# cosdata/cosdata

Hardware: AMD Instinct MI355X
Metric: QPS at recall@10≥0.95, 1024-dim dense cosine, 1/2/4/8 MI355X (higher is better)
Workload: dtype u8

## Files before the change

### cosdata_amd/csrc/engine.hip

```cpp
#include <hip/hip_runtime.h>

#include <algorithm>
#include <cstdarg>
#include <cstdio>
#include <cstdlib>
#include <chrono>
#include <cmath>
#include <condition_variable>
#include <cstring>
#include <map>
#include <mutex>
#include <string>
#include <thread>
#include <vector>

#include "engine_internal.h"

using namespace cosdev;

static thread_local std::string g_err;
int32_t cos_fail(int32_t code, const char *fmt, ...) {
    char buf[512];
    va_list ap;
    va_start(ap, fmt);
    vsnprintf(buf, sizeof(buf), fmt, ap);
    va_end(ap);
    g_err = buf;
    return code;
}

extern "C" const char *cos_last_error_string(void) { return g_err.c_str(); }

extern "C" int32_t cos_device_count(int32_t *out) {
    if (!out) return cos_fail(COS_ERR_INVALID, "null argument");
    int n = 0;
    hipError_t e = hipGetDeviceCount(&n);
    if (e != hipSuccess) { *out = 0; return cos_fail(COS_ERR_NO_DEVICE, "hipGetDeviceCount: %s", hipGetErrorString(e)); }
    *out = n;
    return COS_OK;
}

static u32 pow2ceil(u32 v) { u32 p = 1; while (p < v) p <<= 1; return p; }

int32_t cos_set_device(const cos_index *ix) {
    HIP_TRY(hipSetDevice(ix->p.device));
    return COS_OK;
}

static bool graph_ready(const cos_index *ix) {
// ... 600 lines not shown
                const u32 *row = &adj[(size_t)v * M];
                for (u32 j = M; j-- > 0;) {
                    const u32 u = row[j];
                    if (u != cosdev::ROW_EMPTY && u < n && !seen[u]) stack.push_back(u);
                }
            }
        };
        dfs_from(n - 1);
        for (u32 v = 0; v < n; v++) if (!seen[v]) dfs_from(v);
        HIP_TRY(ix->d_order_rank[kl].alloc(n));
        HIP_TRY(hipMemcpy(ix->d_order_rank[kl], rank.data(), (size_t)n * 4, hipMemcpyHostToDevice));
        ix->order_rank_n[kl] = n;
    }
    ix->order_rank_valid = true;
    return COS_OK;
}

static void clear_current_table(cos_index *ix) {
    ix->d_tcodes = nullptr;
    ix->d_tmags = nullptr;
    ix->d_tcsums = nullptr;
    ix->table_cols = 0;
    ix->table_level_min = 0;
    ix->table_stride = 0;
}
static u32 walk_table_max_cols(const cos_index *ix) {
    const long long env = cosdev::tune_or(cosdev::TUNE_WALK_TABLE_COLS, -1);
    return env >= 0 ? (u32)std::min<long long>(env, 1ll << 20) : ix->walk_table_max_cols;
}
static u32 walk_table_min_B(const cos_index *ix) {
    const long long env = cosdev::tune_or(cosdev::TUNE_WALK_TABLE_MIN_B, -1);
    return env >= 0 ? (u32)std::min<long long>(env, 0xFFFFFFFFll) : ix->walk_table_min_B;
}
static constexpr long long WALK_TABLE_EARLY_WGS_DEFAULT = 0;
static constexpr long long WALK_UP_TABLE_DEFAULT = 1;
cosdev::WalkPlanIn cos_walk_plan_in(const cos_index *ix, u32 B, u32 ef) {
    cosdev::WalkPlanIn in{};
    in.eng = ix->eng;
    in.storage = ix->p.storage;
    in.nchunks = ix->nchunks;
    in.G = ix->G;
    in.num_layers = ix->p.num_layers;
    for (u32 l = 0; l <= ix->p.num_layers; l++) in.M[l] = ix->lv[l].M;
    in.shortlist = ix->p.shortlist_size;
    in.visited_mode = ix->p.visited_mode;
    in.mdim = ix->meta.mdim;
    in.B = B;
    in.ef = ef;
    in.chain = true;
    const long long lat = cosdev::tune_or(cosdev::TUNE_WALK_LAT, -1), lat4 = cosdev::tune_or(cosdev::TUNE_WALK_LAT4, -1);
    in.lat_max_B = lat >= 0 ? (u32)std::min(lat, 0xFFFFFFFFll) : ix->lat_max_B;
    in.lat4_max_B = lat4 >= 0 ? (u32)std::min(lat4, 0xFFFFFFFFll) : ix->lat4_max_B;
    in.small_table_tk = cosdev::tune_or(cosdev::TUNE_WALK_SMALL_TABLE_TK, 1) != 0;
    in.adj_mag_mode = (u32)cosdev::tune_or(cosdev::TUNE_WALK_ADJ_MAG, 1);
    in.table_min_B = walk_table_min_B(ix);
    in.order_min_B = ix->walk_order_min_B;
    in.chain_min_B = ix->chain_min_B;
    in.side_min_B = ix->walk_side_min_B;
    in.table_after_sort = cosdev::tune_or(cosdev::TUNE_WALK_TABLE_AFTER_SORT, 1);
    in.table_supported = cosdev::level_table_eng_supported(ix->eng, ix->row_stride);
    in.adj_mag_valid = ix->adj_mag_valid;
    in.up_table_mode = (u32)std::min<long long>(std::max<long long>(cosdev::tune_or(cosdev::TUNE_WALK_UP_TABLE, WALK_UP_TABLE_DEFAULT), 0), 2);
    in.table_early_wgs = (u32)std::min<long long>(std::max<long long>(cosdev::tune_or(cosdev::TUNE_WALK_TABLE_EARLY_WGS, WALK_TABLE_EARLY_WGS_DEFAULT), 0), 0xFFFFFFFFll);
    in.table_queue = cosdev::level_table_gemm_queue(ix->eng, ix->row_stride);
    in.n_cus = ix->n_cus;
    return in;
}
static int32_t ensure_level_table(cos_index *ix) {
    const u32 max_cols = walk_table_max_cols(ix);
    const bool automatic = max_cols == COS_WALK_TABLE_AUTO;
    const u32 efs = ix->p.ef_search, Mup = ix->p.neighbors_count;
    const u64 c_rule = (u64)cosdev::tune_or(cosdev::TUNE_WALK_TABLE_RULE_C, 2u * efs <= 3u * Mup ? 10 : (efs <= 2u * Mup ? 8 : 6));
    const u64 per_level = automatic ? std::min<u64>(c_rule * ix->p.ef_search * ix->p.neighbors_count, 1u << 20) : (u64)(1u << 20);
    const u64 total_cap = automatic ? (u64)(1u << 20) : (u64)max_cols;
    const u64 key = automatic ? (0x8000000000000000ull | per_level) : (u64)max_cols;
    if (ix->level_table_valid && ix->table_built_for_key == key) return COS_OK;
    if (!ix->level_table_valid) {
        HIP_TRY(hipDeviceSynchronize());
        ix->table_sets.clear();
    }
    ix->level_table_valid = true;
    ix->table_built_for_key = key;
    clear_current_table(ix);
    for (const auto &t : ix->table_sets)
        if (t.key == key) {
            ix->table_level_min = t.level_min;
            ix->table_cols = t.cols;
            ix->table_stride = t.stride;
            memcpy(ix->table_col0, t.col0, sizeof(t.col0));
            ix->d_tcodes = t.tcodes;
            ix->d_tmags = t.tmags;
            ix->d_tcsums = t.tcsums;
            return COS_OK;
        }
    if (!cosdev::level_table_eng_supported(ix->eng, ix->row_stride) || max_cols == 0) return COS_OK;
    const u32 Ltop = ix->p.num_layers;
    u32 cols = 0, lmin = 0;
    for (u32 l = Ltop; l >= 1; l--) {
// ... 158 lines not shown
    u32 ef = 0, visited_mode = 0;
    bool timed = false;
    u64 tab_stride = 0;
    u32 tab_col0[cosdev::MAX_LEVELS] = {};
    const uint8_t *tcodes = nullptr;
    const float *tmags = nullptr;
    const u32 *tcsums = nullptr;
    u32 n_keys = 0, key_level[cosdev::MAX_LEVELS], key_n[cosdev::MAX_LEVELS];
    const u32 *order_rank[cosdev::MAX_LEVELS];
};

static int32_t get_workspace(cos_index *ix, void *key, hipStream_t st, u32 B, u32 top_k, bool host_api, Workspace **out, SearchLaunch *L,
                             bool chain = true) {
    std::lock_guard<std::mutex> g(ix->mu);
    std::unique_ptr<Workspace> &slot = ix->ws[key];
    if (!slot) slot.reset(new Workspace());
    Workspace *w = slot.get();
    const u32 L1 = ix->p.num_layers + 1;
    if (B > w->capB) {
        u32 cap = std::max(B, 64u);
        HIP_TRY(hipStreamSynchronize(st));
        w->capB = 0;
        w->cap_topk = 0;
        HIP_TRY(w->q_codes.alloc((size_t)cap * ix->row_stride));
        HIP_TRY(w->q_mags.alloc(cap));
        HIP_TRY(w->q_raw_mags.alloc(cap));
        HIP_TRY(w->walk_ids.alloc((size_t)cap * L1 * KEEP_SEARCH));
        HIP_TRY(w->walk_sims.alloc((size_t)cap * L1 * KEEP_SEARCH));
        HIP_TRY(w->walk_counts.alloc((size_t)cap * L1));
        HIP_TRY(w->walk_status.alloc(cap));
        HIP_TRY(w->stats.alloc((size_t)cap * 4));
        HIP_TRY(w->stats2.alloc((size_t)cap * 4));
        HIP_TRY(w->qsums.alloc(cap));
        HIP_TRY(w->tab_queue.alloc(16));
        if (ix->eng == ENG_Q2) HIP_TRY(w->qdig.alloc((size_t)cap * (ix->row_stride / 16) * 64));
        HIP_TRY(w->fin_flags.alloc((size_t)cap + 1));
        HIP_TRY(w->rerank_rows.alloc(cap));
        HIP_TRY(w->d_queries.alloc((size_t)cap * ix->p.dim));
        HIP_TRY(w->d_out_counts.alloc(cap));
        HIP_TRY(w->d_out_status.alloc(cap));
        w->capB = cap;
    }
    L->ef = ix->p.ef_search;
    L->visited_mode = ix->p.visited_mode;
    L->timed = ix->timing;
    cosdev::WalkPlanIn in = cos_walk_plan_in(ix, B, L->ef);
    in.chain = chain;
    const cosdev::WalkPlan want = cosdev::walk_plan(in);
    cosdev::WalkHave have{};
    if (want.refill_adj_mag) {
        if (int32_t rc = ensure_adj_mags(ix)) return rc;
        in.adj_mag_valid = ix->adj_mag_valid;
    }
    if (want.prepare_order) {
        if (w->order.cap < w->capB) {
            HIP_TRY(hipStreamSynchronize(st));
            HIP_TRY(cosdev::walk_order_reserve(w->order, w->capB));
        }
        if (int32_t rc = ensure_order_rank(ix)) return rc;
        have.order_buffers = w->order.cap >= B;
        have.n_order_keys = (u32)ix->order_levels.size();
        have.order_level0 = have.n_order_keys ? ix->order_levels[0] : 0u;
    }
    if (want.prepare_table) {
        if (int32_t rc = ensure_level_table(ix)) return rc;
        if (int32_t rc = ensure_adj_up(ix)) return rc;
        have.adj_up_level = ix->adj_up_level;
        const size_t need = (size_t)w->capB * ix->table_stride;
        if (need > w->tab.cap) {
            const size_t budget = (size_t)cosdev::tune_or(cosdev::TUNE_WALK_TABLE_MAX_BYTES, (long long)48 << 30);
            HIP_TRY(hipStreamSynchronize(st));
            ix->table_bytes_total -= w->tab.cap * 4;
            w->tab.reset();
            if (ix->table_bytes_total + need * 4 <= budget) {
                if (const hipError_t e = w->tab.alloc(need); e == hipSuccess)
                    ix->table_bytes_total += need * 4;
                else if (e == hipErrorOutOfMemory)
                    (void)hipGetLastError();
                else
                    HIP_TRY(e);
            }
        }
        have.table_level_min = ix->level_table_valid ? ix->table_level_min : 0u;
        have.table_cols = ix->table_cols;
        have.table_buffer = w->tab && (size_t)B * ix->table_stride <= w->tab.cap;
    }
    L->plan = cosdev::walk_plan(in, &have);
    if (L->plan.use_table) {
        L->tab_stride = ix->table_stride;
        memcpy(L->tab_col0, ix->table_col0, sizeof(L->tab_col0));
        L->tcodes = ix->d_tcodes;
        L->tmags = ix->d_tmags;
        L->tcsums = ix->d_tcsums;
    }
    if (L->plan.ordered)
        for (u32 l : ix->order_levels) {
            L->key_level[L->n_keys] = l;
            L->key_n[L->n_keys] = ix->order_rank_n[l];
            L->order_rank[L->n_keys++] = ix->d_order_rank[l];
        }
    if (host_api && (size_t)top_k * w->capB > (size_t)w->cap_topk * w->capB) {
        w->cap_topk = 0;
        HIP_TRY(w->d_out_ids.alloc((size_t)w->capB * top_k));
        HIP_TRY(w->d_out_scores.alloc((size_t)w->capB * top_k));
        w->cap_topk = top_k;
    }
    if (w->ev.empty()) {
        w->ev.assign((size_t)Workspace::EV_RING * Workspace::EV_PER, nullptr);
        for (auto &e : w->ev) HIP_TRY(hipEventCreate(&e));
    }
    if (!w->walk_done) HIP_TRY(hipEventCreateWithFlags(&w->walk_done, hipEventDisableTiming));
    if (!w->walk_fin) HIP_TRY(hipEventCreateWithFlags(&w->walk_fin, hipEventDisableTiming));
    if (!w->last_range) HIP_TRY(hipEventCreateWithFlags(&w->last_range, hipEventDisableTiming));
    if (!w->upper_done) HIP_TRY(hipEventCreateWithFlags(&w->upper_done, hipEventDisableTiming));
    *out = w;
    return COS_OK;
}

static int32_t run_search(cos_index *ix, Workspace *w, const SearchLaunch &L, const float *d_queries, u32 B, u32 top_k, u32 *d_out_ids,
// ... 1 lines not shown
                          hipStream_t st_fin = nullptr, hipEvent_t walk_ev = nullptr) {
    const cosdev::WalkPlan &plan = L.plan;
    const bool timed = L.timed, ordered = plan.ordered, chained = plan.chained;
    const u32 ef = L.ef, n_keys = L.n_keys;
    IndexDev dev = cos_make_index_dev(ix);
    dev.visited_mode = L.visited_mode;
    for (u32 l = 0; l <= dev.num_layers; l++)
        if (!((plan.use_adj_mag >> l) & 1u)) dev.lv[l].adj_mag = nullptr;
    for (u32 l = 0; l <= dev.num_layers; l++)
        if (plan.up_table_level != l || l == 0u || dev.lv[l].adj_mag == nullptr) dev.lv[l].adj_up = nullptr;
    WalkArgs wa;
    memset(&wa, 0, sizeof(wa));
    if (dev.visited_mode == COS_VISITED_EXACT) {
        int32_t rc = vis_tab_prepare(w->vis, ix, B, ef, st, wa);
        if (rc) return rc;
    }
    hipEvent_t *ev = &w->ev[(size_t)(w->ev_count % Workspace::EV_RING) * Workspace::EV_PER];
    if (timed) HIP_TRY(hipEventRecord(ev[0], st));
    HIP_TRY(launch_quantize_rows(ix->eng, d_queries, ix->p.dim, B, ix->p.dim, ix->p.range_lo, ix->p.range_hi, w->q_codes, ix->row_stride,
                                 w->q_mags, w->q_raw_mags, st, plan.use_table && ix->eng == ENG_U8 ? w->qsums.p : nullptr));
    HIP_TRY(hipMemsetAsync(w->stats2, 0, (size_t)B * 32, st));
    if (plan.use_table) {
        auto table_part = [&](hipEvent_t cos_index::*handle_ev, hipEvent_t own_ev, hipEvent_t *marks, u32 wgs, bool first) -> int32_t {
            if (plan.table_waits_for_sort) {
                std::lock_guard<std::mutex> g(ix->chain_mu);
                if (ix->*handle_ev && ix->*handle_ev != own_ev) HIP_TRY(hipStreamWaitEvent(st, ix->*handle_ev, 0));
            }
            if (timed) HIP_TRY(hipEventRecord(marks[0], st));
            HIP_TRY(cosdev::launch_level_table(ix->eng, w->q_codes, w->q_mags, w->qsums, w->qdig, B, L.tcodes, L.tmags, L.tcsums, ix->row_stride, plan.table_cols,
                                               w->tab, L.tab_stride, ix->n_cus, st, w->tab_queue, wgs, first, plan.table_waits_for_sort));
            if (timed) HIP_TRY(hipEventRecord(marks[1], st));
            return COS_OK;
        };
        if (cosdev::level_table_gemm_queue(ix->eng, ix->row_stride)) HIP_TRY(hipMemsetAsync(w->tab_queue, 0, sizeof(u32), st));
        if (plan.table_early_wgs) {
            if (int32_t rc = table_part(&cos_index::chain_upper_ev, w->upper_done, ev + 4, plan.table_early_wgs, true)) return rc;
            if (int32_t rc = table_part(&cos_index::chain_ev, w->walk_done, ev + 8, 0u, false)) return rc;
        } else if (int32_t rc = table_part(&cos_index::chain_last_range_ev, w->last_range, ev + 4, 0u, true))
            return rc;
    }
    if (timed) HIP_TRY(hipEventRecord(ev[1], st));
    wa.qcodes = w->q_codes;
    wa.qmags = w->q_mags;
    wa.B = B;
    wa.ef = ef;
    wa.keep = KEEP_SEARCH;
    wa.out_ids = w->walk_ids;
    wa.out_sims = w->walk_sims;
    wa.out_counts = w->walk_counts;
    wa.out_status = w->walk_status;
    wa.out_stats = w->stats;
    wa.out_stats2 = w->stats2;
    if (plan.use_table) {
        wa.tab = w->tab;
        wa.tab_mags = L.tmags;
        wa.tab_stride = L.tab_stride;
        wa.tab_level_min = plan.table_level_min;
        memcpy(wa.tab_col0, L.tab_col0, sizeof(L.tab_col0));
    }
    hipStream_t sw = st;
    if (plan.side_stream) {
        if (!w->walk_stream) {
            int lo = 0, hi = 0;
            HIP_TRY(hipDeviceGetStreamPriorityRange(&lo, &hi));
            HIP_TRY(hipStreamCreateWithPriority(&w->walk_stream, hipStreamNonBlocking, lo));
            HIP_TRY(hipEventCreateWithFlags(&w->prep_done, hipEventDisableTiming));
        }
// ... 844 lines not shown
```

### cosdata_amd/csrc/kernels_scan.hip

```cpp
#include <hip/hip_runtime.h>

#include <algorithm>
#include <cstdlib>
#include <type_traits>

#include "device_common.h"
#include "flat_scan.h"
#include "tuning.h"
#include "walk_plan.h"

#ifndef COS_SCAN_MASKED_TU
#define COS_SCAN_MASKED_TU 0
#endif

using namespace cosdev;

namespace {

typedef int i32x4 __attribute__((ext_vector_type(4)));
typedef int i32x16 __attribute__((ext_vector_type(16)));

__device__ __forceinline__ u32 q2_dword_perm(uint4 raw , int pp, int jj) {
    const u32 w0 = pp < 2 ? raw.x : raw.y, w1 = pp < 2 ? raw.z : raw.w;
    const int sh = 4 * (pp & 1) + jj;
    const u32 x0 = w0 >> sh, x1 = sh ? (w1 >> (sh - 1)) : (w1 << 1);
    return (x0 & 0x01010101u) | (x1 & 0x02020202u);
}
__device__ __forceinline__ uint4 q2_piece_perm(uint4 raw, int pp) {
    return make_uint4(q2_dword_perm(raw, pp, 0), q2_dword_perm(raw, pp, 1), q2_dword_perm(raw, pp, 2), q2_dword_perm(raw, pp, 3));
}


__device__ __forceinline__ u32 q2_nibble_dword(uint4 raw, int pp, int jj);
template <int ENG>
struct ScanRow;
template <>
struct ScanRow<ENG_Q2> {
    typedef uint4 Raw;
    static __device__ __forceinline__ Raw zero() { return make_uint4(0, 0, 0, 0); }
    static __device__ __forceinline__ bool in_row(u32 j, u64 row_stride) { return (u64)j * 16 < row_stride; }
    static __device__ __forceinline__ Raw load(const uint8_t *__restrict__ rowp, int j, u64) { return *(const uint4 *)(rowp + (u64)j * 16); }
// ... 643 lines not shown
                        const float q4 = acc[i][r];
                        if (row < B && __builtin_fmaf(q4, rx, -T[i][r]) >= 0.0f && scan_live<MASKED>(fo.m, row, n0 + colx)) {
                            const u32 dot = (u32)(q4 * 4.0f);
                            const u32 sp = atomicAdd(stage_cnt, 1u);
                            if (sp < AREG_STAGE) {
                                stage[3 * sp] = colx;
                                stage[3 * sp + 1] = row;
                                stage[3 * sp + 2] = dot;
                            } else
                                areg_append(fo, qmags, mags, metric, n0, colx, row, dot);
                        }
                    }
                }
            }
        });
        __syncthreads();
    };
    while (true) {
        tile_body(std::integral_constant<int, 0>{}, t);
        t += G;
        if (t >= n_tiles) break;
        tile_body(std::integral_constant<int, 1>{}, t);
        t += G;
        if (t >= n_tiles) break;
    }
    const u32 staged = min(*stage_cnt, (u32)AREG_STAGE);
    for (u32 e = tid; e < staged; e += 512) areg_append(fo, qmags, mags, metric, n0, stage[3 * e], stage[3 * e + 1], stage[3 * e + 2]);
}

template <int KC, bool Q2>
__global__ __launch_bounds__(256) void level_table_areg(const uint8_t *__restrict__ qcodes ,
                                                        const u32 *__restrict__ qsums, u32 B, const uint8_t *__restrict__ tcodes,
                                                        const u32 *__restrict__ tcsums, u64 row_stride , u32 ncols,
                                                        float *__restrict__ tab, u64 tab_stride, u32 *__restrict__ queue, u32 stripe) {
    constexpr int K = KC * 64, KS = KC * 2, LDB = K + 16;
    constexpr int PC = Q2 ? KC : K / 16;
    constexpr int NP = (64 * PC + 255) / 256;
    extern __shared__ __attribute__((aligned(16))) unsigned char areg_lds[];
    __shared__ u32 s_item;
    const int tid = threadIdx.x, lane = tid & 63, w = tid >> 6, half = lane >> 5, l31 = lane & 31;
    const u32 n_tiles = (ncols + 63) / 64, row_groups = (B + 255) / 256, n_items = (n_tiles + stripe - 1) / stripe * row_groups;
    u32 row0 = 0, rg_now = 0xFFFFFFFFu, t = 0, t_end = 0;
    i32x4 a[2][KS];
    int rqs[2][16];
    auto load_rows = [&]() __attribute__((always_inline)) {
        static_for<0, 2 * KS>([&](auto Ic) __attribute__((always_inline)) {
            constexpr int i = decltype(Ic)::value / KS, s = decltype(Ic)::value % KS;
            const u32 row = row0 + 32 * i + l31;
            i32x4 v = *(const i32x4 *)(qcodes + (u64)(row < B ? row : B - 1) * K + 32 * s + 16 * half);
            if constexpr (!Q2) v = v ^ (int)0x80808080;
            a[i][s] = row < B ? v : i32x4{0, 0, 0, 0};
            asm volatile("" : "+a"(a[i][s]));
        });
#pragma unroll
        for (int i = 0; i < 2; i++)
#pragma unroll
            for (int r = 0; r < 16; r++) {
                const u32 row = row0 + 32 * i + (r & 3) + 8 * (r >> 2) + 4 * half;
                rqs[i][r] = Q2 ? 0 : 128 * (int)qsums[row < B ? row : B - 1] - 16384 * K;
            }
    };
    uint4 raw[NP];
    auto load_tile = [&](u32 tile) __attribute__((always_inline)) {
#pragma unroll
        for (int p = 0; p < NP; p++) {
            const u32 g = (u32)p * 256u + (u32)tid, gg = g < 64u * PC ? g : 0u, c = gg / (u32)PC, pc = gg % (u32)PC;
            const u32 col = tile * 64 + c, cc = col < ncols ? col : ncols - 1;
            raw[p] = *(const uint4 *)(tcodes + (u64)cc * row_stride + (u64)pc * 16);
        }
    };
    auto store_tile = [&](int buf) __attribute__((always_inline)) {
#pragma unroll
        for (int p = 0; p < NP; p++) {
            const u32 g = (u32)p * 256u + (u32)tid, c = g / (u32)PC, pc = g % (u32)PC;
            if (64 * PC % 256 != 0 && g >= 64u * PC) continue;
            unsigned char *dst = areg_lds + (size_t)buf * 64 * LDB + (size_t)c * LDB;
            if constexpr (Q2) {
#pragma unroll
                for (int pp = 0; pp < 4; pp++) *(uint4 *)(dst + (size_t)pc * 64 + pp * 16) = q2_piece_perm(raw[p], pp);
            } else {
                uint4 v = raw[p];
                v.x ^= 0x80808080u; v.y ^= 0x80808080u; v.z ^= 0x80808080u; v.w ^= 0x80808080u;
                *(uint4 *)(dst + (size_t)pc * 16) = v;
            }
        }
    };
    while (true) {
        __syncthreads();
        if (tid == 0) s_item = atomicAdd(queue, 1u);
        __syncthreads();
        const u32 item = s_item;
        if (item >= n_items) break;
        const u32 rg = item % row_groups;
        t = item / row_groups * stripe;
        t_end = min(n_tiles, t + stripe);
        if (rg != rg_now) {
            rg_now = rg;
            row0 = rg * 256 + w * 64;
            load_rows();
        }
        load_tile(t);
        store_tile(0);
        __syncthreads();
        int P = 0;
        while (true) {
            const bool more = t + 1 < t_end;
            if (more) load_tile(t + 1);
            const unsigned char *bt = areg_lds + (size_t)P * 64 * LDB + l31 * LDB + 16 * half;
            i32x16 acc[2][2];
            i32x4 bf[3][2];
#pragma unroll
            for (int s = 0; s < 2 && s < KS; s++) {
                bf[s][0] = *(const i32x4 *)(bt + 32 * s);
                bf[s][1] = *(const i32x4 *)(bt + 32 * LDB + 32 * s);
            }
            static_for<0, KS>([&](auto Sc) __attribute__((always_inline)) {
                constexpr int s = decltype(Sc)::value;
                if (s + 2 < KS) {
                    bf[(s + 2) % 3][0] = *(const i32x4 *)(bt + 32 * (s + 2));
                    bf[(s + 2) % 3][1] = *(const i32x4 *)(bt + 32 * LDB + 32 * (s + 2));
                }
                __builtin_amdgcn_sched_barrier(0);
                const i32x4 b0 = bf[s % 3][0], b1 = bf[s % 3][1];
                areg_mfma<s == 0>(acc[0][0], a[0][s], b0);
                areg_mfma<s == 0>(acc[0][1], a[0][s], b1);
                areg_mfma<s == 0>(acc[1][0], a[1][s], b0);
                areg_mfma<s == 0>(acc[1][1], a[1][s], b1);
                __builtin_amdgcn_sched_barrier(0);
            });
            auto epilogue = [&](auto fullc) __attribute__((always_inline)) {
                constexpr bool FULL = decltype(fullc)::value;
#pragma unroll
                for (int j = 0; j < 2; j++) {
                    const u32 col = t * 64 + 32 * j + l31;
                    const bool cv = FULL || col < ncols;
                    int cs = 0;
                    if constexpr (!Q2) cs = 128 * (int)tcsums[cv ? col : ncols - 1];
#pragma unroll
                    for (int i = 0; i < 2; i++) {
                        const u32 rbase = row0 + 32 * i + 4 * half;
                        float *out = tab + (u64)rbase * tab_stride + col;
#pragma unroll
                        for (int r = 0; r < 16; r++) {
                            const u32 dr = (r & 3) + 8 * (r >> 2);
                            const u32 dot = (u32)(acc[i][j][r] + rqs[i][r] + cs);
                            if (FULL || (cv && rbase + dr < B)) out[(u64)dr * tab_stride] = (float)dot;
                        }
                    }
                }
            };
            if (row0 + 64 <= B && t * 64 + 64 <= ncols) epilogue(std::true_type{});
            else epilogue(std::false_type{});
            if (!more) break;
            store_tile(P ^ 1);
            __syncthreads();
            P ^= 1;
            t += 1;
        }
    }
}

template <int KC, int RB , bool MASKED = false>
__global__ __launch_bounds__(256) void flat_scan_u8_areg(const uint8_t *__restrict__ qcodes , const u32 *__restrict__ qsums,
                                                         const float *__restrict__ qmags, u32 B, const uint8_t *__restrict__ codes,
                                                         const u32 *__restrict__ csums, const float *__restrict__ mags, u64 row_stride, u32 n0,
                                                         u32 n_chunk, u32 metric, const FusedOut fo) {
    constexpr int K = KC * 64, KS = KC * 2, LDB = K + 16, PC = K / 16, NP = (64 * PC + 255) / 256;
    extern __shared__ __attribute__((aligned(16))) unsigned char areg_lds[];
    u32 *stage = (u32 *)(areg_lds + (size_t)2 * 64 * LDB), *stage_cnt = stage + 3 * AREG_STAGE;
    const int tid = threadIdx.x, lane = tid & 63, w = tid >> 6, half = lane >> 5, l31 = lane & 31;
    const u32 row0 = blockIdx.y * (128 * RB) + w * (32 * RB);
    const u32 n_tiles = (n_chunk + 63) / 64, G = gridDim.x;
    u32 t = blockIdx.x;
    if (t >= n_tiles) return;
    if (tid == 0) *stage_cnt = 0;
    i32x4 a[RB][KS];
    static_for<0, RB * KS>([&](auto Ic) __attribute__((always_inline)) {
        constexpr int i = decltype(Ic)::value / KS, s = decltype(Ic)::value % KS;
        const u32 row = row0 + 32 * i + l31;
        i32x4 v = *(const i32x4 *)(qcodes + (u64)(row < B ? row : B - 1) * K + 32 * s + 16 * half);
        v = v ^ (int)0x80808080;
        a[i][s] = row < B ? v : i32x4{0, 0, 0, 0};
        asm volatile("" : "+a"(a[i][s]));
    });
    int rqs[RB][16];
    float T[RB][16];
#pragma unroll
    for (int i = 0; i < RB; i++)
#pragma unroll
        for (int r = 0; r < 16; r++) {
            const u32 row = row0 + 32 * i + (r & 3) + 8 * (r >> 2) + 4 * half, rc = row < B ? row : B - 1;
// ... 201 lines not shown
    hipError_t e = hipFuncSetAttribute((const void *)flat_scan_u8_areg<KC, RB, M>, hipFuncAttributeMaxDynamicSharedMemorySize, (int)lds);
    if (e != hipSuccess) return e;
    const dim3 grid(std::min((nc + 63) / 64, n_cus), (B + 128 * RB - 1) / (128 * RB));
    hipLaunchKernelGGL((flat_scan_u8_areg<KC, RB, M>), grid, dim3(256), lds, st, qcodes, qsums, qmags, B, codes, csums, mags, row_stride, n0, nc, metric, fo);
    return hipGetLastError();
}
#if COS_SCAN_MASKED_TU
hipError_t launch_flat_scan_u8_masked(u32 kdims, u32 n_cus, hipStream_t st, const uint8_t *qcodes, const u32 *qsums, const float *qmags, u32 B, const uint8_t *codes,
                                      const u32 *csums, const float *mags, u64 row_stride, u32 n0, u32 nc, u32 metric, const FusedOut &fo) {
#else
hipError_t launch_flat_scan_u8_masked(u32 kdims, u32 n_cus, hipStream_t st, const uint8_t *qcodes, const u32 *qsums, const float *qmags, u32 B, const uint8_t *codes,
                                      const u32 *csums, const float *mags, u64 row_stride, u32 n0, u32 nc, u32 metric, const FusedOut &fo);
hipError_t launch_flat_scan_u8(u32 kdims, u32 n_cus, hipStream_t st, const uint8_t *qcodes, const u32 *qsums, const float *qmags, u32 B, const uint8_t *codes,
                               const u32 *csums, const float *mags, u64 row_stride, u32 n0, u32 nc, u32 metric, const FusedOut &fo) {
    if (fo.m.bits) return launch_flat_scan_u8_masked(kdims, n_cus, st, qcodes, qsums, qmags, B, codes, csums, mags, row_stride, n0, nc, metric, fo);
#endif
#define U8_CASE(KC) case KC: return launch_u8_kc<KC, SCAN_M>(n_cus, st, qcodes, qsums, qmags, B, codes, csums, mags, row_stride, n0, nc, metric, fo)
    switch (kdims / 64) {
        U8_CASE(2); U8_CASE(4); U8_CASE(6); U8_CASE(8); U8_CASE(12); U8_CASE(16);
        default: return hipErrorInvalidValue;
    }
#undef U8_CASE
}

#if !COS_SCAN_MASKED_TU

bool level_table_areg_supported(int eng, u64 row_stride) {
    if (eng == ENG_U8) return row_stride % 64 == 0 && flat_scan_supported((u32)row_stride);
    if (eng == ENG_Q2) return row_stride % 16 == 0 && flat_scan_supported((u32)(row_stride / 16) * 64);
    return false;
}
template <int KC, bool Q2>
static hipError_t launch_table_kc(u32 wgs, hipStream_t st, const uint8_t *qcodes, const u32 *qsums, u32 B, const uint8_t *tcodes, const u32 *tcsums,
                                  u64 row_stride, u32 ncols, float *tab, u64 tab_stride, u32 *queue, u32 stripe) {
    const size_t lds = (size_t)2 * 64 * (KC * 64 + 16);
    hipError_t e = hipFuncSetAttribute((const void *)level_table_areg<KC, Q2>, hipFuncAttributeMaxDynamicSharedMemorySize, (int)lds);
    if (e != hipSuccess) return e;
    hipLaunchKernelGGL((level_table_areg<KC, Q2>), dim3(wgs), dim3(256), lds, st, qcodes, qsums, B, tcodes, tcsums, row_stride, ncols, tab, tab_stride, queue, stripe);
    return hipGetLastError();
}
hipError_t launch_level_table_areg(int eng, u32 n_cus, hipStream_t st, const uint8_t *qcodes, const u32 *qsums, u32 B, const uint8_t *tcodes, const u32 *tcsums,
                                   u64 row_stride, u32 ncols, float *tab, u64 tab_stride, u32 *queue, u32 wgs, bool shared) {
    const u32 stripe = table_gemm_stripe_tiles(B, ncols, n_cus, shared), n_items = table_gemm_items(B, ncols, n_cus, shared);
    wgs = std::max(1u, std::min(n_items, wgs ? wgs : std::max(1u, n_cus)));
    const u32 kc = eng == ENG_Q2 ? (u32)(row_stride / 16) : (u32)(row_stride / 64);
#define TAB_CASE(KC)                                                                                                                                  \
    case KC:                                                                                                                                          \
        return eng == ENG_Q2 ? launch_table_kc<KC, true>(wgs, st, qcodes, qsums, B, tcodes, tcsums, row_stride, ncols, tab, tab_stride, queue, stripe) \
                             : launch_table_kc<KC, false>(wgs, st, qcodes, qsums, B, tcodes, tcsums, row_stride, ncols, tab, tab_stride, queue, stripe)
    switch (kc) {
        TAB_CASE(2); TAB_CASE(4); TAB_CASE(6); TAB_CASE(8); TAB_CASE(12); TAB_CASE(16);
        default: return hipErrorInvalidValue;
    }
#undef TAB_CASE
}

hipError_t launch_flat_scan_expand_queries(int eng, const uint8_t *qcodes, u64 row_stride, u32 B, u32 kdims, uint8_t *digits, hipStream_t st, bool fp4) {
    const dim3 grid((u32)(((u64)B * (kdims / 64) + 255) / 256));
    if (fp4) {
        if (eng == ENG_Q2) hipLaunchKernelGGL(expand_q2_nibbles_kernel<ENG_Q2>, grid, dim3(256), 0, st, qcodes, row_stride, B, kdims, digits);
        else if (eng == ENG_Q1) hipLaunchKernelGGL(expand_q2_nibbles_kernel<ENG_Q1>, grid, dim3(256), 0, st, qcodes, row_stride, B, kdims, digits);
        else return hipErrorInvalidValue;
        return hipGetLastError();
    }
    if (eng == ENG_Q2) hipLaunchKernelGGL(expand_q2_digits_perm_kernel<ENG_Q2>, grid, dim3(256), 0, st, qcodes, row_stride, B, kdims, digits);
    else if (eng == ENG_Q1) hipLaunchKernelGGL(expand_q2_digits_perm_kernel<ENG_Q1>, grid, dim3(256), 0, st, qcodes, row_stride, B, kdims, digits);
    else if (eng == ENG_Q3) hipLaunchKernelGGL(expand_q2_digits_perm_kernel<ENG_Q3>, grid, dim3(256), 0, st, qcodes, row_stride, B, kdims, digits);
    else return hipErrorInvalidValue;
    return hipGetLastError();
}
#endif

}
```

### cosdata_amd/csrc/walk_plan.h

```cpp
#pragma once
#include <algorithm>
#include <cstdint>

namespace cosdev {

constexpr int WALK_PLAN_MAX_LEVELS = 16;
constexpr int WALK_PLAN_ENG_U8 = 0, WALK_PLAN_ENG_Q2 = 1;
constexpr uint32_t WALK_PLAN_FAST_MAX_EF = 1024u;

constexpr uint32_t ADJ_MAG_REFILL_MIN_B = 1024u, ADJ_MAG_USE_MIN_B = 4096u;

enum class WalkKernel : uint8_t {
    General,
    Throughput,
    Lat1,
    Lat4
};

struct WalkPlanIn {
    int eng;
    uint32_t storage;
    uint32_t nchunks, G;
    uint32_t num_layers, M[WALK_PLAN_MAX_LEVELS], shortlist, visited_mode, mdim;
    uint32_t B, ef;
// ... 20 lines not shown
    bool order_buffers;
    uint32_t adj_up_level;
};

struct WalkPlan {
    WalkKernel kernel;
    bool ordered;
    bool use_table;
    bool table_waits_for_sort;
    uint32_t table_early_wgs;
    uint32_t use_adj_mag;
    bool refill_adj_mag;
    bool chained;
    bool side_stream;
    bool prepare_order, prepare_table;
    uint32_t table_level_min, table_cols, cut_after_level;
    uint32_t up_table_level;
};

inline uint32_t table_gemm_stripe_tiles(uint32_t B, uint32_t cols, uint32_t n_cus, bool shared) {
    const uint32_t n_tiles = (cols + 63u) / 64u, row_groups = (B + 255u) / 256u, cus = n_cus ? n_cus : 256u;
    if (!shared) {
        const uint32_t groups = std::max(1u, cus / std::max(1u, std::min(row_groups, cus)));
        return std::max(1u, (n_tiles + groups - 1u) / groups);
    }
    const uint64_t units = (uint64_t)n_tiles * row_groups;
    return (uint32_t)std::min<uint64_t>(64u, std::max<uint64_t>(2u, units / (24ull * cus)));
}
inline uint32_t table_gemm_items(uint32_t B, uint32_t cols, uint32_t n_cus, bool shared) {
    const uint32_t n_tiles = (cols + 63u) / 64u, st = table_gemm_stripe_tiles(B, cols, n_cus, shared);
    return (uint32_t)std::min<uint64_t>(0xFFFFFFFFull, (uint64_t)((n_tiles + st - 1u) / st) * ((B + 255u) / 256u));
}

inline bool walk_rows_over_64_slots(const WalkPlanIn &in) {
    for (uint32_t l = 0; l <= in.num_layers; l++)
        if (std::min(in.M[l], in.shortlist) > 64u) return true;
    return false;
}

inline bool walk_general_needed(const WalkPlanIn &in) {
    if (in.ef > WALK_PLAN_FAST_MAX_EF) return true;
    if (in.nchunks != 0u && in.G != 0u && (in.nchunks + in.G - 1u) / in.G > (in.storage == 0u  ? 4u : 1u)) return true;
    return walk_rows_over_64_slots(in);
}

inline bool walk_latency_domain(const WalkPlanIn &in, uint32_t max_B) {
    if (max_B == 0 || in.B > max_B) return false;
    if (in.visited_mode != 0) return false;
    if (in.eng != WALK_PLAN_ENG_U8 && in.eng != WALK_PLAN_ENG_Q2) return false;
    if (in.nchunks == 0 || in.nchunks > 64u) return false;
    if (in.ef == 0 || in.ef > 256) return false;
    return true;
}

inline WalkKernel walk_fast_kernel(const WalkPlanIn &in, bool table_available) {
    if (in.no_self_seed) return WalkKernel::Throughput;
    const bool lat4 = walk_latency_domain(in, in.lat4_max_B) && std::max(in.M[0], in.M[in.num_layers]) <= 64u;
    if (table_available && in.small_table_tk && in.eng == WALK_PLAN_ENG_U8)
        return in.ef > 128u && lat4 ? WalkKernel::Lat4 : WalkKernel::Throughput;
    if (lat4) return WalkKernel::Lat4;
    if (walk_latency_domain(in, in.lat_max_B)) return WalkKernel::Lat1;
    return WalkKernel::Throughput;
}

inline WalkPlan walk_plan(const WalkPlanIn &in, const WalkHave *have = nullptr) {
    WalkPlan p{};
    const bool general = walk_general_needed(in);
    p.ordered = !general && in.order_min_B && in.B >= in.order_min_B && in.ef <= 256u && (!have || (have->n_order_keys > 0 && have->order_buffers));
    bool table = !general && in.table_min_B && (have ? have->table_level_min != 0 && have->table_buffer : in.table_supported);
    const bool table_size = in.B >= in.table_min_B || in.B <= in.lat4_max_B;
    if (general) p.kernel = WalkKernel::General;
    else if (p.ordered) {
        p.kernel = WalkKernel::Throughput;
        table = table && table_size;
    } else {
        const WalkKernel with_table = walk_fast_kernel(in, true);
        table = table && ((with_table == WalkKernel::Lat4 && in.eng == WALK_PLAN_ENG_U8) || (with_table == WalkKernel::Throughput && table_size));
        p.kernel = table ? with_table : walk_fast_kernel(in, false);
    }
    p.use_table = table;
    p.chained = in.chain && in.B >= in.chain_min_B;
    if (have && table) {
        p.table_level_min = have->table_level_min;
        p.table_cols = have->table_cols;
        p.table_waits_for_sort = p.chained && (in.table_after_sort == 2 || (in.table_after_sort == 1 && (uint64_t)have->table_cols * in.B >= (1ull << 30)));
        if (p.table_waits_for_sort && in.table_queue)
            p.table_early_wgs = std::min(in.table_early_wgs, table_gemm_items(in.B, have->table_cols, in.n_cus, true));
    }
    if (have && p.ordered) p.cut_after_level = have->order_level0;
    if (in.adj_mag_valid && in.adj_mag_mode != 0)
        for (uint32_t l = 0; l <= in.num_layers; l++)
            if (in.adj_mag_mode == 2 || (in.ef <= 2u * in.M[l] && in.B >= ADJ_MAG_USE_MIN_B)) p.use_adj_mag |= 1u << l;
    p.refill_adj_mag = !in.adj_mag_valid && in.B >= ADJ_MAG_REFILL_MIN_B;
    if (have && p.use_table && p.kernel == WalkKernel::Throughput && in.up_table_mode != 0 && in.eng == WALK_PLAN_ENG_U8 && in.G == 64u &&
        in.mdim == 0u && have->table_level_min >= 2u && have->adj_up_level == have->table_level_min - 1u) {
        const uint32_t l = have->table_level_min - 1u;
        if (in.up_table_mode == 2 && in.adj_mag_valid && in.adj_mag_mode != 0) p.use_adj_mag |= 1u << l;
        if ((p.use_adj_mag >> l) & 1u) p.up_table_level = l;
    }
    p.side_stream = in.side_min_B && in.B >= in.side_min_B;
    p.prepare_order = p.ordered;
    p.prepare_table = p.use_table;
    return p;
}

}
```

Baseline: 1.124 million.

## Pipeline work claims in level table GEMM and shard the queue per row group

Restructures the persistent level_table_areg kernel so each workgroup claims its next work item while still computing the current one. It also loads the next item's first tile across item boundaries instead of synchronising and re-claiming at the top of every item. A new claim helper can optionally split the single atomic work counter into one counter per 256-row group, with fallback to the other counters, to cut atomic contention and keep query rows resident longer. It also adds an auto mode for the early-workgroup count, but the default ratio of zero makes it resolve to zero. The cost is a more complex double-buffered claim protocol and more queue words to clear on each search.

```diff
diff --git a/cosdata_amd/csrc/engine.hip b/cosdata_amd/csrc/engine.hip
--- a/cosdata_amd/csrc/engine.hip
+++ b/cosdata_amd/csrc/engine.hip
@@ -15,6 +15,7 @@
 #include <vector>
 
 #include "engine_internal.h"
+#include "table_claim.h"
 
 using namespace cosdev;
 
@@ -681,7 +682,8 @@
     const long long env = cosdev::tune_or(cosdev::TUNE_WALK_TABLE_MIN_B, -1);
     return env >= 0 ? (u32)std::min<long long>(env, 0xFFFFFFFFll) : ix->walk_table_min_B;
 }
-static constexpr long long WALK_TABLE_EARLY_WGS_DEFAULT = 0;
+static constexpr long long WALK_TABLE_EARLY_WGS_DEFAULT = -1;
+static long long walk_table_early_knob() { return cosdev::tune_or(cosdev::TUNE_WALK_TABLE_EARLY_WGS, WALK_TABLE_EARLY_WGS_DEFAULT); }
 static constexpr long long WALK_UP_TABLE_DEFAULT = 1;
 cosdev::WalkPlanIn cos_walk_plan_in(const cos_index *ix, u32 B, u32 ef) {
     cosdev::WalkPlanIn in{};
@@ -710,9 +712,9 @@
     in.table_supported = cosdev::level_table_eng_supported(ix->eng, ix->row_stride);
     in.adj_mag_valid = ix->adj_mag_valid;
     in.up_table_mode = (u32)std::min<long long>(std::max<long long>(cosdev::tune_or(cosdev::TUNE_WALK_UP_TABLE, WALK_UP_TABLE_DEFAULT), 0), 2);
-    in.table_early_wgs = (u32)std::min<long long>(std::max<long long>(cosdev::tune_or(cosdev::TUNE_WALK_TABLE_EARLY_WGS, WALK_TABLE_EARLY_WGS_DEFAULT), 0), 0xFFFFFFFFll);
     in.table_queue = cosdev::level_table_gemm_queue(ix->eng, ix->row_stride);
     in.n_cus = ix->n_cus;
+    in.table_early_wgs = cosdev::table_early_wgs_resolve(walk_table_early_knob(), in, ix->level_table_valid ? ix->table_cols : 0u);
     return in;
 }
 static int32_t ensure_level_table(cos_index *ix) {
@@ -937,7 +939,7 @@
         HIP_TRY(w->stats.alloc((size_t)cap * 4));
         HIP_TRY(w->stats2.alloc((size_t)cap * 4));
         HIP_TRY(w->qsums.alloc(cap));
-        HIP_TRY(w->tab_queue.alloc(16));
+        HIP_TRY(w->tab_queue.alloc(std::max(16u, cosdev::table_queue_words(cap))));
         if (ix->eng == ENG_Q2) HIP_TRY(w->qdig.alloc((size_t)cap * (ix->row_stride / 16) * 64));
         HIP_TRY(w->fin_flags.alloc((size_t)cap + 1));
         HIP_TRY(w->rerank_rows.alloc(cap));
@@ -990,6 +992,7 @@
         have.table_cols = ix->table_cols;
         have.table_buffer = w->tab && (size_t)B * ix->table_stride <= w->tab.cap;
     }
+    in.table_early_wgs = cosdev::table_early_wgs_resolve(walk_table_early_knob(), in, have.table_cols);
     L->plan = cosdev::walk_plan(in, &have);
     if (L->plan.use_table) {
         L->tab_stride = ix->table_stride;
@@ -1057,7 +1060,8 @@
             if (timed) HIP_TRY(hipEventRecord(marks[1], st));
             return COS_OK;
         };
-        if (cosdev::level_table_gemm_queue(ix->eng, ix->row_stride)) HIP_TRY(hipMemsetAsync(w->tab_queue, 0, sizeof(u32), st));
+        if (cosdev::level_table_gemm_queue(ix->eng, ix->row_stride))
+            HIP_TRY(hipMemsetAsync(w->tab_queue, 0, sizeof(u32) * cosdev::table_queue_words(B), st));
         if (plan.table_early_wgs) {
             if (int32_t rc = table_part(&cos_index::chain_upper_ev, w->upper_done, ev + 4, plan.table_early_wgs, true)) return rc;
             if (int32_t rc = table_part(&cos_index::chain_ev, w->walk_done, ev + 8, 0u, false)) return rc;
diff --git a/cosdata_amd/csrc/kernels_scan.hip b/cosdata_amd/csrc/kernels_scan.hip
--- a/cosdata_amd/csrc/kernels_scan.hip
+++ b/cosdata_amd/csrc/kernels_scan.hip
@@ -7,6 +7,7 @@
 #include "device_common.h"
 #include "flat_scan.h"
 #include "tuning.h"
+#include "table_claim.h"
 #include "walk_plan.h"
 
 #ifndef COS_SCAN_MASKED_TU
@@ -716,15 +717,17 @@
 __global__ __launch_bounds__(256) void level_table_areg(const uint8_t *__restrict__ qcodes ,
                                                         const u32 *__restrict__ qsums, u32 B, const uint8_t *__restrict__ tcodes,
                                                         const u32 *__restrict__ tcsums, u64 row_stride , u32 ncols,
-                                                        float *__restrict__ tab, u64 tab_stride, u32 *__restrict__ queue, u32 stripe) {
+                                                        float *__restrict__ tab, u64 tab_stride, u32 *__restrict__ queue, u32 stripe,
+                                                        bool per_group ) {
     constexpr int K = KC * 64, KS = KC * 2, LDB = K + 16;
     constexpr int PC = Q2 ? KC : K / 16;
     constexpr int NP = (64 * PC + 255) / 256;
     extern __shared__ __attribute__((aligned(16))) unsigned char areg_lds[];
-    __shared__ u32 s_item;
+    __shared__ u32 s_claim[2];
     const int tid = threadIdx.x, lane = tid & 63, w = tid >> 6, half = lane >> 5, l31 = lane & 31;
-    const u32 n_tiles = (ncols + 63) / 64, row_groups = (B + 255) / 256, n_items = (n_tiles + stripe - 1) / stripe * row_groups;
-    u32 row0 = 0, rg_now = 0xFFFFFFFFu, t = 0, t_end = 0;
+    const u32 n_tiles = (ncols + 63) / 64;
+    const TableQueueShape qs = table_queue_shape(B, ncols, stripe, per_group);
+    u32 row0 = 0;
     i32x4 a[2][KS];
     int rqs[2][16];
     auto load_rows = [&]() __attribute__((always_inline)) {
@@ -769,78 +772,99 @@
             }
         }
     };
+    TableClaim claim = table_claim_start(blockIdx.x, qs);
+    auto claim_into = [&](u32 slot) __attribute__((always_inline)) {
+        s_claim[slot] = table_claim_next(claim, qs, [&](u32 c) { return atomicAdd(queue + c, 1u); });
+    };
+    auto item_tiles = [&](u32 item, u32 &rg, u32 &t0, u32 &t1) __attribute__((always_inline)) {
+        u32 sidx;
+        table_item_decode(item, qs, rg, sidx);
+        t0 = sidx * stripe;
+        t1 = min(n_tiles, t0 + stripe);
+    };
+    if (tid == 0) claim_into(0u);
+    __syncthreads();
+    const u32 item0 = (u32)__builtin_amdgcn_readfirstlane((int)s_claim[0]);
+    if (item0 == TABLE_CLAIM_NONE) return;
+    u32 n = 0, rg_now, t, t_end;
+    item_tiles(item0, rg_now, t, t_end);
+    row0 = rg_now * 256 + w * 64;
+    load_rows();
+    load_tile(t);
+    store_tile(0);
+    if (tid == 0 && t + 1 >= t_end) claim_into(1u);
+    __syncthreads();
+    int P = 0;
     while (true) {
-        __syncthreads();
-        if (tid == 0) s_item = atomicAdd(queue, 1u);
-        __syncthreads();
-        const u32 item = s_item;
-        if (item >= n_items) break;
-        const u32 rg = item % row_groups;
-        t = item / row_groups * stripe;
-        t_end = min(n_tiles, t + stripe);
-        if (rg != rg_now) {
-            rg_now = rg;
-            row0 = rg * 256 + w * 64;
-            load_rows();
-        }
-        load_tile(t);
-        store_tile(0);
-        __syncthreads();
-        int P = 0;
-        while (true) {
-            const bool more = t + 1 < t_end;
-            if (more) load_tile(t + 1);
-            const unsigned char *bt = areg_lds + (size_t)P * 64 * LDB + l31 * LDB + 16 * half;
-            i32x16 acc[2][2];
-            i32x4 bf[3][2];
-#pragma unroll
-            for (int s = 0; s < 2 && s < KS; s++) {
-                bf[s][0] = *(const i32x4 *)(bt + 32 * s);
-                bf[s][1] = *(const i32x4 *)(bt + 32 * LDB + 32 * s);
-            }
-            static_for<0, KS>([&](auto Sc) __attribute__((always_inline)) {
-                constexpr int s = decltype(Sc)::value;
-                if (s + 2 < KS) {
-                    bf[(s + 2) % 3][0] = *(const i32x4 *)(bt + 32 * (s + 2));
-                    bf[(s + 2) % 3][1] = *(const i32x4 *)(bt + 32 * LDB + 32 * (s + 2));
-                }
-                __builtin_amdgcn_sched_barrier(0);
-                const i32x4 b0 = bf[s % 3][0], b1 = bf[s % 3][1];
-                areg_mfma<s == 0>(acc[0][0], a[0][s], b0);
-                areg_mfma<s == 0>(acc[0][1], a[0][s], b1);
-                areg_mfma<s == 0>(acc[1][0], a[1][s], b0);
-                areg_mfma<s == 0>(acc[1][1], a[1][s], b1);
-                __builtin_amdgcn_sched_barrier(0);
-            });
-            auto epilogue = [&](auto fullc) __attribute__((always_inline)) {
-                constexpr bool FULL = decltype(fullc)::value;
-#pragma unroll
-                for (int j = 0; j < 2; j++) {
-                    const u32 col = t * 64 + 32 * j + l31;
-                    const bool cv = FULL || col < ncols;
-                    int cs = 0;
-                    if constexpr (!Q2) cs = 128 * (int)tcsums[cv ? col : ncols - 1];
-#pragma unroll
-                    for (int i = 0; i < 2; i++) {
-                        const u32 rbase = row0 + 32 * i + 4 * half;
-                        float *out = tab + (u64)rbase * tab_stride + col;
-#pragma unroll
-                        for (int r = 0; r < 16; r++) {
-                            const u32 dr = (r & 3) + 8 * (r >> 2);
-                            const u32 dot = (u32)(acc[i][j][r] + rqs[i][r] + cs);
-                            if (FULL || (cv && rbase + dr < B)) out[(u64)dr * tab_stride] = (float)dot;
-                        }
+        const bool last = t + 1 >= t_end;
+        u32 nx_rg = rg_now, nx_t = t + 1, nx_end = t_end;
+        bool more = true;
+        if (last) {
+            const u32 nx = (u32)__builtin_amdgcn_readfirstlane((int)s_claim[(n + 1u) & 1u]);
+            more = nx != TABLE_CLAIM_NONE;
+            if (more) item_tiles(nx, nx_rg, nx_t, nx_end);
+        }
+        if (more) {
+            load_tile(nx_t);
+            if (tid == 0 && nx_t + 1 >= nx_end) claim_into((n + (last ? 2u : 1u)) & 1u);
+        }
+        const unsigned char *bt = areg_lds + (size_t)P * 64 * LDB + l31 * LDB + 16 * half;
+        i32x16 acc[2][2];
+        i32x4 bf[3][2];
+#pragma unroll
+        for (int s = 0; s < 2 && s < KS; s++) {
+            bf[s][0] = *(const i32x4 *)(bt + 32 * s);
+            bf[s][1] = *(const i32x4 *)(bt + 32 * LDB + 32 * s);
+        }
+        static_for<0, KS>([&](auto Sc) __attribute__((always_inline)) {
+            constexpr int s = decltype(Sc)::value;
+            if (s + 2 < KS) {
+                bf[(s + 2) % 3][0] = *(const i32x4 *)(bt + 32 * (s + 2));
+                bf[(s + 2) % 3][1] = *(const i32x4 *)(bt + 32 * LDB + 32 * (s + 2));
+            }
+            __builtin_amdgcn_sched_barrier(0);
+            const i32x4 b0 = bf[s % 3][0], b1 = bf[s % 3][1];
+            areg_mfma<s == 0>(acc[0][0], a[0][s], b0);
+            areg_mfma<s == 0>(acc[0][1], a[0][s], b1);
+            areg_mfma<s == 0>(acc[1][0], a[1][s], b0);
+            areg_mfma<s == 0>(acc[1][1], a[1][s], b1);
+            __builtin_amdgcn_sched_barrier(0);
+        });
+        auto epilogue = [&](auto fullc) __attribute__((always_inline)) {
+            constexpr bool FULL = decltype(fullc)::value;
+#pragma unroll
+            for (int j = 0; j < 2; j++) {
+                const u32 col = t * 64 + 32 * j + l31;
+                const bool cv = FULL || col < ncols;
+                int cs = 0;
+                if constexpr (!Q2) cs = 128 * (int)tcsums[cv ? col : ncols - 1];
+#pragma unroll
+                for (int i = 0; i < 2; i++) {
+                    const u32 rbase = row0 + 32 * i + 4 * half;
+                    float *out = tab + (u64)rbase * tab_stride + col;
+#pragma unroll
+                    for (int r = 0; r < 16; r++) {
+                        const u32 dr = (r & 3) + 8 * (r >> 2);
+                        const u32 dot = (u32)(acc[i][j][r] + rqs[i][r] + cs);
+                        if (FULL || (cv && rbase + dr < B)) out[(u64)dr * tab_stride] = (float)dot;
                     }
                 }
-            };
-            if (row0 + 64 <= B && t * 64 + 64 <= ncols) epilogue(std::true_type{});
-            else epilogue(std::false_type{});
-            if (!more) break;
-            store_tile(P ^ 1);
-            __syncthreads();
-            P ^= 1;
-            t += 1;
-        }
+            }
+        };
+        if (row0 + 64 <= B && t * 64 + 64 <= ncols) epilogue(std::true_type{});
+        else epilogue(std::false_type{});
+        if (!more) break;
+        if (nx_rg != rg_now) {
+            row0 = nx_rg * 256 + w * 64;
+            load_rows();
+        }
+        if (last) n++;
+        rg_now = nx_rg;
+        t = nx_t;
+        t_end = nx_end;
+        store_tile(P ^ 1);
+        __syncthreads();
+        P ^= 1;
     }
 }
 
@@ -1108,11 +1132,12 @@
 }
 template <int KC, bool Q2>
 static hipError_t launch_table_kc(u32 wgs, hipStream_t st, const uint8_t *qcodes, const u32 *qsums, u32 B, const uint8_t *tcodes, const u32 *tcsums,
-                                  u64 row_stride, u32 ncols, float *tab, u64 tab_stride, u32 *queue, u32 stripe) {
+                                  u64 row_stride, u32 ncols, float *tab, u64 tab_stride, u32 *queue, u32 stripe, bool per_group) {
     const size_t lds = (size_t)2 * 64 * (KC * 64 + 16);
     hipError_t e = hipFuncSetAttribute((const void *)level_table_areg<KC, Q2>, hipFuncAttributeMaxDynamicSharedMemorySize, (int)lds);
     if (e != hipSuccess) return e;
-    hipLaunchKernelGGL((level_table_areg<KC, Q2>), dim3(wgs), dim3(256), lds, st, qcodes, qsums, B, tcodes, tcsums, row_stride, ncols, tab, tab_stride, queue, stripe);
+    hipLaunchKernelGGL((level_table_areg<KC, Q2>), dim3(wgs), dim3(256), lds, st, qcodes, qsums, B, tcodes, tcsums, row_stride, ncols, tab, tab_stride, queue, stripe,
+                       per_group);
     return hipGetLastError();
 }
 hipError_t launch_level_table_areg(int eng, u32 n_cus, hipStream_t st, const uint8_t *qcodes, const u32 *qsums, u32 B, const uint8_t *tcodes, const u32 *tcsums,
@@ -1122,8 +1147,8 @@
     const u32 kc = eng == ENG_Q2 ? (u32)(row_stride / 16) : (u32)(row_stride / 64);
 #define TAB_CASE(KC)                                                                                                                                  \
     case KC:                                                                                                                                          \
-        return eng == ENG_Q2 ? launch_table_kc<KC, true>(wgs, st, qcodes, qsums, B, tcodes, tcsums, row_stride, ncols, tab, tab_stride, queue, stripe) \
-                             : launch_table_kc<KC, false>(wgs, st, qcodes, qsums, B, tcodes, tcsums, row_stride, ncols, tab, tab_stride, queue, stripe)
+        return eng == ENG_Q2 ? launch_table_kc<KC, true>(wgs, st, qcodes, qsums, B, tcodes, tcsums, row_stride, ncols, tab, tab_stride, queue, stripe, shared) \
+                             : launch_table_kc<KC, false>(wgs, st, qcodes, qsums, B, tcodes, tcsums, row_stride, ncols, tab, tab_stride, queue, stripe, shared)
     switch (kc) {
         TAB_CASE(2); TAB_CASE(4); TAB_CASE(6); TAB_CASE(8); TAB_CASE(12); TAB_CASE(16);
         default: return hipErrorInvalidValue;
diff --git a/cosdata_amd/csrc/table_claim.h b/cosdata_amd/csrc/table_claim.h
--- /dev/null
+++ b/cosdata_amd/csrc/table_claim.h
@@ -0,0 +1,62 @@
+#pragma once
+#include <cstdint>
+
+#if defined(__HIPCC__) || defined(__CUDACC__)
+#define COS_CLAIM_FN __host__ __device__ inline
+#else
+#define COS_CLAIM_FN inline
+#endif
+
+namespace cosdev {
+
+constexpr uint32_t TABLE_CLAIM_NONE = 0xFFFFFFFFu;
+
+struct TableQueueShape {
+    uint32_t row_groups, stripes;
+    uint32_t n_counters;
+    uint32_t per_counter;
+    bool per_group;
+};
+
+COS_CLAIM_FN TableQueueShape table_queue_shape(uint32_t B, uint32_t ncols, uint32_t stripe, bool per_group) {
+    TableQueueShape s;
+    const uint32_t n_tiles = (ncols + 63u) / 64u;
+    s.row_groups = (B + 255u) / 256u;
+    s.stripes = (n_tiles + stripe - 1u) / stripe;
+    s.per_group = per_group;
+    s.n_counters = per_group ? s.row_groups : 1u;
+    s.per_counter = per_group ? s.stripes : s.stripes * s.row_groups;
+    return s;
+}
+
+COS_CLAIM_FN uint32_t table_queue_words(uint32_t B) { return B > 256u ? (B + 255u) / 256u : 1u; }
+
+struct TableClaim {
+    uint32_t counter;
+    uint32_t missed;
+};
+
+COS_CLAIM_FN TableClaim table_claim_start(uint32_t block, const TableQueueShape &s) { return TableClaim{s.n_counters ? block % s.n_counters : 0u, 0u}; }
+
+template <class FetchAdd>
+COS_CLAIM_FN uint32_t table_claim_next(TableClaim &c, const TableQueueShape &s, FetchAdd &&fetch_add) {
+    while (c.missed < s.n_counters) {
+        const uint32_t v = fetch_add(c.counter);
+        if (v < s.per_counter) return c.counter * s.per_counter + v;
+        c.missed++;
+        c.counter = c.counter + 1u == s.n_counters ? 0u : c.counter + 1u;
+    }
+    return TABLE_CLAIM_NONE;
+}
+
+COS_CLAIM_FN void table_item_decode(uint32_t item, const TableQueueShape &s, uint32_t &row_group, uint32_t &stripe_idx) {
+    if (s.per_group) {
+        row_group = item / s.stripes;
+        stripe_idx = item % s.stripes;
+    } else {
+        row_group = item % s.row_groups;
+        stripe_idx = item / s.row_groups;
+    }
+}
+
+}
diff --git a/cosdata_amd/csrc/walk_plan.h b/cosdata_amd/csrc/walk_plan.h
--- a/cosdata_amd/csrc/walk_plan.h
+++ b/cosdata_amd/csrc/walk_plan.h
@@ -76,6 +76,24 @@
     return (uint32_t)std::min<uint64_t>(0xFFFFFFFFull, (uint64_t)((n_tiles + st - 1u) / st) * ((B + 255u) / 256u));
 }
 
+inline bool table_gemm_gated(const WalkPlanIn &in, uint32_t table_cols) {
+    const bool chained = in.chain && in.B >= in.chain_min_B;
+    return chained && (in.table_after_sort == 2 || (in.table_after_sort == 1 && (uint64_t)table_cols * in.B >= (1ull << 30)));
+}
+
+constexpr uint32_t TABLE_EARLY_AUTO_RATIO = 0u;
+inline uint32_t table_early_wgs_auto(bool gated_queue, uint32_t B, uint32_t table_cols, uint32_t n_cus, uint32_t ratio = TABLE_EARLY_AUTO_RATIO) {
+    if (!gated_queue || B == 0u || table_cols == 0u || ratio == 0u) return 0u;
+    const uint64_t cus = n_cus ? n_cus : 256u, units = (uint64_t)((table_cols + 63u) / 64u) * ((B + 255u) / 256u);
+    const uint64_t n = (units * cus * ratio + (uint64_t)B * 1024u - 1u) / ((uint64_t)B * 1024u);
+    if (2u * n >= cus) return 0u;
+    return (uint32_t)std::min<uint64_t>(std::max<uint64_t>(n, 1u), table_gemm_items(B, table_cols, n_cus, true));
+}
+inline uint32_t table_early_wgs_resolve(long long knob, const WalkPlanIn &in, uint32_t table_cols, uint32_t ratio = TABLE_EARLY_AUTO_RATIO) {
+    if (knob >= 0) return (uint32_t)std::min<long long>(knob, 0xFFFFFFFFll);
+    return table_early_wgs_auto(in.table_queue && table_gemm_gated(in, table_cols), in.B, table_cols, in.n_cus, ratio);
+}
+
 inline bool walk_rows_over_64_slots(const WalkPlanIn &in) {
     for (uint32_t l = 0; l <= in.num_layers; l++)
         if (std::min(in.M[l], in.shortlist) > 64u) return true;
@@ -127,7 +145,7 @@
     if (have && table) {
         p.table_level_min = have->table_level_min;
         p.table_cols = have->table_cols;
-        p.table_waits_for_sort = p.chained && (in.table_after_sort == 2 || (in.table_after_sort == 1 && (uint64_t)have->table_cols * in.B >= (1ull << 30)));
+        p.table_waits_for_sort = table_gemm_gated(in, have->table_cols);
         if (p.table_waits_for_sort && in.table_queue)
             p.table_early_wgs = std::min(in.table_early_wgs, table_gemm_items(in.B, have->table_cols, in.n_cus, true));
     }
```

Measured after the change: 1.137 million, median of 6. 1.01x the previous value.
